# metasnv-tool/metaSNV

Hardware: AMD Instinct MI355X
Metric: pileup Gbases/s across all samples (higher is better)
Workload: dtype u8

## Files before the change

metasnv_amd/csrc/device.h:

```cpp
#pragma once

#include <cstdint>

#include <string>
#include <vector>

#include "dataset.h"

namespace msnv {

struct Pair32 { uint32_t x, y; };
struct MergedGroupDev { uint64_t hdr_base; uint32_t tile, pair_lo, n_pairs, n_pieces; };

constexpr uint8_t ANN_GENE_MINUS = 1, ANN_GENE_LINEAR = 2;
struct AnnGene   { int64_t start; int32_t contig; uint32_t flags; };
struct AnnContig { int64_t cg_base, cg_len; uint32_t goff, pad; };
struct AnnHost {
    std::vector<uint32_t> seg_beg, seg_end;
    std::vector<int32_t>  seg_gene;
    std::vector<AnnGene>  genes;
    std::vector<AnnContig> contigs;
    std::vector<uint8_t>  codons;
};
struct AnnDev {
    uint32_t *seg_beg = nullptr, *seg_end = nullptr; int32_t *seg_gene = nullptr;
    AnnGene *genes = nullptr; AnnContig *contigs = nullptr; uint8_t *codons = nullptr;
    uint32_t n_seg = 0;
    msnv_site_ann *out = nullptr; uint64_t cap_out = 0;
    uint32_t *err = nullptr;
    bool ready = false;
    std::string key;
    std::vector<std::string> gene_names;
};
int  ann_build(msnv_dataset &ds, const Annotation &an, AnnHost &h);
void ann_gene_names(const Annotation &an, const std::vector<std::string> &contigs, std::vector<std::string> &out);
int  dev_ann_upload(DeviceCols &d, const AnnHost &h);
int  dev_annotate(DeviceCols &d, uint32_t n_sites, uint32_t drop_gpos, void *stream, double *ms, uint32_t err_gpos[2]);

struct DeviceCols {
    ReadHdr  *hdr = nullptr;
    PieceHdr *hdr8 = nullptr;
    uint32_t *hdr4 = nullptr;
    PieceHdr *hdr8m = nullptr;
    uint32_t *tile_pair_merged = nullptr;
    uint32_t  n_work_merged = 0;
    MergedGroupDev *merged_groups = nullptr; uint32_t n_merged_groups = 0;
    uint32_t *blk = nullptr;
    bool      dense = true;
    uint8_t  *seq = nullptr;
    uint8_t  *qual = nullptr;
    uint64_t *s_read_base = nullptr, *s_seq_base = nullptr;
    uint32_t *ref4 = nullptr;
    uint32_t *ref_lc = nullptr;
    TilePair *pairs = nullptr;
    uint32_t *tile_pair_start = nullptr;
    WorkItem *work = nullptr;
    ChunkDesc *chunks = nullptr;
    uint32_t *tile_vbeg = nullptr, *tile_vend = nullptr;
    uint32_t  n_tiles = 0, n_pairs = 0, n_work = 0, n_work_narrow = 0, n_samples = 0;
    uint64_t  n_reads = 0, n_seq_bytes = 0, n_chunks = 0, n_hdr8m = 0, n_blk = 0;
    uint32_t *tot = nullptr;
    uint32_t *active_tiles = nullptr;
    uint32_t  n_active_tiles = 0;
    uint8_t  *part = nullptr;
// ... 144 lines not shown
```

metasnv_amd/csrc/kernels.hip:

```cpp
#include <hip/hip_runtime.h>

#include <algorithm>
#include <cstdio>
#include <cstdlib>
#include <cstring>
#include <mutex>
#include <unordered_map>
#include <vector>

#include "device.h"

namespace msnv {

#define HIP_TRY(expr)                                                                         \
    do {                                                                                      \
        hipError_t e_ = (expr);                                                               \
        if (e_ != hipSuccess) return fail(MSNV_EHIP, "%s failed: %s", #expr, hipGetErrorString(e_)); \
    } while (0)

constexpr int LANES_PER_READ = 8;
static_assert(LANES_PER_READ * 16 == SEG_MAX, "segment pieces are sized for 8 lanes of 16 bases");

struct PileupArgs {
    const ReadHdr  *hdr;
    const uint32_t *blk;
    const PieceHdr *hdr8;
    const uint32_t *hdr4;
    const PieceHdr *hdr8m;
    uint32_t        n_narrow;
    const uint8_t  *seq;
    const uint8_t  *qual;
    const uint64_t *s_read_base, *s_seq_base;
    const uint32_t *ref4;
    const TilePair *pairs;
    const WorkItem *work;
    const ChunkDesc *chunks;
    uint32_t       *tot;
    uint8_t        *part;
    uint64_t        npos;
    uint8_t        *spill;
    uint8_t        *aspill;
    Pair32         *events;   uint32_t cap_events;
    Pair32         *overflow; uint32_t cap_overflow;
    uint32_t       *counters;
    uint32_t       *ev_count;
    uint32_t        min_baseq;
    uint32_t       *ind4;
    uint32_t       *unc_bits;
    uint32_t       *slot_dirty;
    uint32_t        min_snvs;
    uint32_t        n_fused_lo;
    int             min_cov; double min_frac;
    const uint32_t *ref_lc, *tile_vbeg, *tile_vend, *tile_stage_idx;
    TileStage      *tile_stage;
    uint32_t       *stage_ovf;
};

__device__ __forceinline__ uint32_t allele_index(uint32_t code) {
    return (code == 1u) ? 0u : (code == 2u) ? 1u : (code == 4u) ? 2u : (code == 8u) ? 3u : 4u;
}
__device__ __forceinline__ uint32_t nz_bytes(uint32_t x) {
    return (((x & 0x7f7f7f7fu) + 0x7f7f7f7fu) | x) & 0x80808080u;
}
__device__ __forceinline__ uint32_t count_nz_bytes(const uint4 a, const uint4 b) {
    return (uint32_t)__popc(nz_bytes(a.x) | nz_bytes(a.y) >> 1 | nz_bytes(a.z) >> 2 | nz_bytes(a.w) >> 3 |
                            nz_bytes(b.x) >> 4 | nz_bytes(b.y) >> 5 | nz_bytes(b.z) >> 6 | nz_bytes(b.w) >> 7);
}
__device__ __forceinline__ uint32_t nz_nibbles(uint32_t x) {
    return (((x & 0x77777777u) + 0x77777777u) | x) & 0x88888888u;
}
__device__ __forceinline__ uint32_t nibflags_to_bits(uint32_t f) {
    const uint32_t e = f & 0x08080808u, o = (f >> 4) & 0x08080808u;
    return (__builtin_amdgcn_udot4(o, 0x80200802u, __builtin_amdgcn_udot4(e, 0x40100401u, 0u, false), false)) >> 3;
}
__device__ __forceinline__ uint4 any_uint4() {
    uint4 v;
    asm volatile("" : "=v"(v.x), "=v"(v.y), "=v"(v.z), "=v"(v.w));
    return v;
}
__device__ __forceinline__ uint2 lowq_fetch(const uint8_t *qlow, const uint64_t bit) {
    uint2 v;
    __builtin_memcpy(&v, qlow + (bit >> 3), 8);
    return v;
}
__device__ __forceinline__ uint32_t lowq_bits(const uint2 v, const uint32_t shift) {
    return (uint32_t)(((unsigned long long)v.y << 32 | v.x) >> shift);
}

template <int CTRL, int ROW_MASK>
__device__ __forceinline__ int dpp_add(int x) {
    return x + __builtin_amdgcn_update_dpp(0, x, CTRL, ROW_MASK, 0xf, false);
}
__device__ __forceinline__ int wave_inclusive_scan(int x) {
    x = dpp_add<0x111, 0xf>(x);
    x = dpp_add<0x112, 0xf>(x);
    x = dpp_add<0x114, 0xf>(x);
    x = dpp_add<0x118, 0xf>(x);
    x = dpp_add<0x142, 0xa>(x);
    x = dpp_add<0x143, 0xc>(x);
    return x;
}

__device__ __forceinline__ uint32_t tot_mode_of(const WorkItem &w) { return (w.part_lo >> 1) & 3u; }
__device__ __forceinline__ void tot_add(uint32_t *tot, const uint32_t mode, const uint32_t t0, const uint32_t p, const uint32_t n0, const uint32_t n1,
                                        const uint32_t n2, const uint32_t n3) {
    uint32_t *base = tot + 4ull * t0;
    if (mode == 0u) atomicAdd(base + p, n0 | n1 << 8 | n2 << 16 | n3 << 24);
    else if (mode == 1u) {
        if (n0 | n1) atomicAdd(base + 2u * p, n0 | n1 << 16);
        if (n2 | n3) atomicAdd(base + 2u * p + 1u, n2 | n3 << 16);
    } else {
        if (n0) atomicAdd(base + 4u * p, n0);
        if (n1) atomicAdd(base + 4u * p + 1u, n1);
        if (n2) atomicAdd(base + 4u * p + 2u, n2);
        if (n3) atomicAdd(base + 4u * p + 3u, n3);
    }
}
__device__ __forceinline__ void tot_add_one(uint32_t *tile_tot, const uint32_t mode, const uint32_t p, const uint32_t x, const uint32_t n) {
    const uint32_t shpack = mode == 0u ? 0x18100800u : mode == 1u ? 0x10001000u : 0u;
    const uint32_t byte_off = ((p << mode) + (x >> (2u - mode))) * 4u;
// ... 227 lines not shown
    *reinterpret_cast<uint2 *>(&L.start[2 * tid]) = make_uint2(0u, 0u);
    *reinterpret_cast<uint2 *>(&L.end[2 * tid]) = make_uint2(0u, 0u);
    L.exc[EXC_PAD + tid] = 0ull;
    if (lane == 0) L.carry[wave] = 0u;
    if (tid == 0) L.end[TILE / 4] = 0;
    const int mine = (int)(__builtin_amdgcn_udot4(st.x, 0x01010101u, __builtin_amdgcn_udot4(st.y, 0x01010101u, 0u, false), false)) -
                     (int)(__builtin_amdgcn_udot4(en.x, 0x01010101u, __builtin_amdgcn_udot4(en.y, 0x01010101u, 0u, false), false));
    d += wave_inclusive_scan(mine) - mine;
    const uint32_t v0 = ((uint32_t)d + st.x - en.x) * 0x01010101u;
    const uint32_t v1 = ((v0 >> 24) + st.y - en.y) * 0x01010101u;
    const uint32_t c0 = v0 - ex.x, c1 = v1 - ex.y;
    tc[0] += c0 & 0x00ff00ffu; tc[1] += (c0 >> 8) & 0x00ff00ffu;
    tc[2] += c1 & 0x00ff00ffu; tc[3] += (c1 >> 8) & 0x00ff00ffu;
    if (!MERGED) *reinterpret_cast<uint2 *>(a.spill + (uint64_t)k * TILE + N_PPT * tid) = make_uint2(c0, c1);
    if (MERGED && FUSED) {
        *reinterpret_cast<uint2 *>(&L.start[2 * tid]) = make_uint2(c0, c1);
        return;
    }
    if constexpr (DA && !MERGED) {
        uint32_t *row = reinterpret_cast<uint32_t *>(a.aspill) + (uint64_t)k * TILE + N_PPT * tid;
        const uint32_t ge = (0x80u - min(a.min_snvs, 127u)) * 0x01010101u;
#pragma unroll
        for (uint32_t half = 0; half < 2u; ++half) {
            const uint4 v = *reinterpret_cast<uint4 *>(&L.al[N_PPT * tid + 4u * half]);
            const uint32_t w4[4] = {v.x, v.y, v.z, v.w};
            *reinterpret_cast<uint4 *>(row + 4u * half) = v;
            if (!(v.x | v.y | v.z | v.w)) continue;
            *reinterpret_cast<uint4 *>(&L.al[N_PPT * tid + 4u * half]) = make_uint4(0u, 0u, 0u, 0u);
            dirty = true;
            uint32_t todo = 0;
#pragma unroll
            for (uint32_t j = 0; j < 4u; ++j) todo |= (split ? w4[j] != 0u : ((((w4[j] & 0x7f7f7f7fu) + ge) | w4[j]) & 0x80808080u) != 0u) ? 1u << j : 0u;
            while (todo) {
                const uint32_t j = (uint32_t)__builtin_ctz(todo);
                todo &= todo - 1u;
                const uint32_t word = j == 0u ? w4[0] : j == 1u ? w4[1] : j == 2u ? w4[2] : w4[3];
                const uint32_t gpos = t0 + N_PPT * tid + 4u * half + j;
#pragma unroll
                for (uint32_t x = 0; x < 4u; ++x) {
                    const uint32_t n = (word >> (8u * x)) & 0xffu;
                    if (n >= a.min_snvs) atomicOr(&a.ind4[gpos >> 3], 1u << (4u * (gpos & 7u) + x));
                    else if (n && split) atomicOr(&a.unc_bits[gpos >> 5], 1u << (gpos & 31u));
                }
            }
        }
        return;
    }
    uint32_t pm = 0, myev;
    {
        const uint4 a0 = *reinterpret_cast<uint4 *>(&L.al[N_PPT * tid]);
        const uint4 a1 = *reinterpret_cast<uint4 *>(&L.al[N_PPT * tid + 4]);
        const uint32_t alw[N_PPT] = {a0.x, a0.y, a0.z, a0.w, a1.x, a1.y, a1.z, a1.w};
#pragma unroll
        for (int j = 0; j < N_PPT; ++j) pm |= (alw[j] ? 1u : 0u) << j;
        myev = count_nz_bytes(a0, a1);
    }
    if (!__any(pm != 0u)) return;
    dirty |= pm != 0u;
    if (MERGED) {
        while (pm) {
            const uint32_t j = (uint32_t)__builtin_ctz(pm);
            pm &= pm - 1u;
            const uint32_t word = L.al[N_PPT * tid + j];
            L.al[N_PPT * tid + j] = 0u;
            const uint32_t gpos = t0 + N_PPT * tid + j;
            for (uint32_t m = nz_bytes(word); m; m &= m - 1u) {
                const uint32_t x = (uint32_t)__builtin_ctz(m) >> 3;
                const uint32_t n = (word >> (8u * x)) & 0xffu;
                tot_add_one(a.tot + 4ull * t0, tmode, N_PPT * tid + j, x, n);
                if (n >= a.min_snvs) atomicOr(&a.unc_bits[gpos >> 5], 1u << (gpos & 31u));
            }
        }
        return;
    }
    const uint32_t ei = (uint32_t)wave_inclusive_scan((int)myev);
    uint32_t res = 0;
    if (lane == 63 && ei) {
        uint32_t cur = atomicAdd(&L.evn, 0u);
        for (;;) {
            if (cur + ei > (uint32_t)N_EVCAP) { res = 0x80000000u | atomicAdd(a.ev_count, ei); break; }
            const uint32_t seen = atomicCAS(&L.evn, cur, cur + ei);
            if (seen == cur) { res = cur; break; }
            cur = seen;
        }
    }
    res = (uint32_t)__builtin_amdgcn_readlane((int)res, 63);
    const bool direct = (res & 0x80000000u) != 0u;
    uint32_t slot = (res & 0x7fffffffu) + ei - myev;
    while (pm) {
        const uint32_t j = (uint32_t)__builtin_ctz(pm);
        pm &= pm - 1u;
        const uint32_t word = L.al[N_PPT * tid + j];
        L.al[N_PPT * tid + j] = 0u;
        const uint32_t gpos = t0 + N_PPT * tid + j;
        for (uint32_t m = nz_bytes(word); m; m &= m - 1u) {
            const uint32_t x = (uint32_t)__builtin_ctz(m) >> 3;
            const uint32_t n = (word >> (8u * x)) & 0xffu;
            tot_add_one(a.tot + 4ull * t0, tmode, N_PPT * tid + j, x, n);
            if (n >= a.min_snvs) atomicOr(&a.ind4[gpos >> 3], 1u << (4u * (gpos & 7u) + x));
            else if (split) atomicOr(&a.unc_bits[gpos >> 5], 1u << (gpos & 31u));
            const Pair32 e{gpos, sample << 18 | x << 16 | n};
            if (direct) { if (slot < a.cap_events) a.events[slot] = e; }
            else L.ev[slot] = e;
            ++slot;
        }
    }
}

// ... 561 lines not shown
        desc_refill(L.desc, a.chunks + w.chunk_lo, c, nch, tid);
        if (L.evn >= (uint32_t)(N_EVCAP / 2)) flush_events<DenseLds, N_NT, N_EVCAP>(L, a, tid);

        const uint8_t *seq = a.seq + cd.seq_base;
        const uint64_t qbit0 = 2ull * cd.seq_base;
        uint4 sq[ROUNDS]; uint2 ql[ROUNDS];
#pragma unroll
        for (int r = 0; r < ROUNDS; ++r) {
            const uint32_t b = (uint32_t)(r * N_NT + tid);
            sq[r] = any_uint4(); ql[r] = make_uint2(0u, 0u);
            if (b < nblk) {
                ql[r] = lowq_fetch(a.qual, qbit0 + 32ull * b);
                sq[r] = *reinterpret_cast<const uint4 *>(seq + 16ull * b);
            }
        }
#pragma unroll
        for (int r = 0; r < ROUNDS; ++r) {
            if (!__any((uint32_t)(r * N_NT + tid) < nblk)) continue;
            const uint32_t d = dcur[r];
            const uint32_t P0A = d & 2047u, nA = (d >> 11) & 63u, PBv = (d >> 17) & 0xfffu;
            const bool hasB = PBv != BLK_NO_B;
            const uint32_t sB = (nA + 1u) & ~1u;
            if (d & BLK_START_A) atomicAdd(&L.start[P0A >> 2], 1u << (8u * (P0A & 3u)));
            if (d & BLK_END_A) { const uint32_t e = P0A + nA; atomicAdd(&L.end[e >> 2], 1u << (8u * (e & 3u))); }
            if (d != BLK_EMPTY && (P0A >> 9) != ((P0A + nA) >> 9)) atomicAdd(&L.carry[(P0A + nA) >> 9], 1u);
            if (hasB) {
                const uint32_t s = PBv + sB - 32u;
                if ((s >> 9) != (PBv >> 9)) atomicAdd(&L.carry[PBv >> 9], 1u);
                atomicAdd(&L.start[s >> 2], 1u << (8u * (s & 3u)));
                if (d & BLK_END_B) { const uint32_t e = PBv; atomicAdd(&L.end[e >> 2], 1u << (8u * (e & 3u))); }
            }
            const uint32_t lq = lowq_bits(ql[r], (uint32_t)qbit0 & 7u);
            dense_segment(L, sq[r], lq, P0A + 32u, 0, (int)nA);
            if (__any(hasB)) dense_segment(L, sq[r], lq, hasB ? PBv : 32u, hasB ? (int)sB : 32, 32);
        }
        if (last_chunk) {
            __syncthreads();
            narrow_pass<DenseLds, D_PAD>(L, a, tc, dirty, t0, tid, lane, wave, cd.sample, cd.pair, cd.pad, tot_mode_of(w));
        }
    }
    __syncthreads();
    flush_events<DenseLds, N_NT, N_EVCAP>(L, a, tid);
    store_part_row(a.part, w, tc, tid);
    store_item_dirty(a.slot_dirty, w, dirty, tid);
}

constexpr int GATE_NT = 256;
constexpr int GATE_PPT = TILE / GATE_NT;
static_assert(GATE_PPT == 8, "the gate kernel is written for 8 positions per thread (one site_bits word per 8 lanes)");

struct CellMap { const uint32_t *tile_site_base; const unsigned long long *tile_cell_base; const uint32_t *tile_nslots; unsigned long long cap_cells;
                 const unsigned long long *block_row; };
__device__ __forceinline__ uint64_t cell_of(const CellMap &m, const uint32_t tile, const uint32_t site, const uint32_t slot) {
    return m.tile_cell_base[tile] + (uint64_t)(site - m.tile_site_base[tile]) * m.tile_nslots[tile] + slot;
}

template <int NT>
__device__ __forceinline__ void zero_span(uint8_t *p, const uint64_t n, const uint32_t tid) {
    const uint64_t head = min(n, (uint64_t)((16u - (uint32_t)(reinterpret_cast<uintptr_t>(p) & 15u)) & 15u));
    if ((uint64_t)2u * tid < head) *reinterpret_cast<uint16_t *>(p + 2u * tid) = 0;
    uint8_t *q = p + head;
    const uint64_t body = (n - head) >> 4;
    const uint4 z = make_uint4(0u, 0u, 0u, 0u);
    for (uint64_t i = tid; i < body; i += NT) reinterpret_cast<uint4 *>(q)[i] = z;
    const uint64_t tail0 = head + (body << 4);
    if (tail0 + 2u * tid < n) *reinterpret_cast<uint16_t *>(p + tail0 + 2u * tid) = 0;
}

template <int NT>
__device__ __forceinline__ void zero_cells(uint16_t *ncol, uint16_t *cov_col, const unsigned long long cap_cells, const unsigned long long first, const unsigned long long n, const uint32_t tid) {
    if (n <= (unsigned long long)NT) {
        if (tid < (uint32_t)n) {
#pragma unroll
            for (int x = 0; x < 4; ++x) ncol[(uint64_t)x * cap_cells + first + tid] = 0;
            cov_col[first + tid] = 0;
        }
        return;
    }
#pragma unroll
    for (int x = 0; x < 4; ++x) zero_span<NT>(reinterpret_cast<uint8_t *>(ncol + (uint64_t)x * cap_cells + first), n * sizeof(uint16_t), tid);
    zero_span<NT>(reinterpret_cast<uint8_t *>(cov_col + first), n * sizeof(uint16_t), tid);
}

struct GateTile { uint32_t tile, slot_lo, slot_16, slot_w, slot_hi, vbeg, vend, n_slots; uint64_t row0; uint32_t tot_mode, staged, pair_lo, n_plane_pairs, pad0, pad1; };

struct GateArgs {
    uint32_t *tot; const uint8_t *part; const uint64_t *slot_off; const uint32_t *tile_slot_start, *tile_slot_u16, *tile_slot_wide; uint64_t npos;
    const uint32_t *tile_vbeg, *tile_vend; int min_cov, min_snvs; double min_frac;
    uint32_t *ind4, *unc_bits;
    const uint32_t *ref4, *ref_lc;
    unsigned long long *site_bits; uint32_t *site_rank; SiteRec *sites; uint32_t cap_sites; uint32_t *counters, *counters_next;
    uint32_t *tile_site_base, *tile_site_cnt; const uint32_t *active_tiles;
    uint16_t *ncol; uint16_t *cov_col; uint8_t *site_flags; uint32_t cap_out;
    const uint32_t *tile_nslots; unsigned long long *tile_cell_base; unsigned long long cap_cells;
    const GateTile *gate_tiles; uint32_t *tile_dirty; uint32_t *unc_sites; uint32_t use_dirty; unsigned long long *block_row;
    uint8_t *site_elig; uint32_t any_split;
    uint32_t n_active, tiles_per_wg;
    const TileStage *tile_stage;
    const uint8_t *aspill;
    uint32_t zero_next;
    const uint32_t *tile_list;
    uint32_t solo_cells;
};

constexpr uint32_t GATE_STAGE = 384;
constexpr uint32_t GATE_MAX_TILES = 8;
struct GateStageTile { uint32_t tile, site_rel, total, n_slots; unsigned long long cell_rel; };
// ... 560 lines not shown
                uint32_t v[4], c[4];
#pragma unroll
                for (uint32_t u = 0; u < 4u; ++u) {
                    const uint32_t k = min(kl + 4u * u, kB - 1u);
                    v[u] = rows[(uint64_t)k * TILE + off];
                    c[u] = (a.pairs[ps + k].pad >> 8) - GA_SLOTS * b;
                }
#pragma unroll
                for (uint32_t u = 0; u < 4u; ++u) {
                    if (kl + 4u * u >= kB || v[u] == 0u) continue;
#pragma unroll
                    for (uint32_t x = 0; x < 4u; ++x) {
                        const uint32_t n = (v[u] >> (8u * x)) & 0xffu;
                        if (n) atomicAdd(&s_acc[lane * GA_ROW + x * (GA_SLOTS / 2u) + (c[u] >> 1)], n << (16u * (c[u] & 1u)));
                    }
                }
            }
            __syncthreads();
            for (uint32_t idx = tid; idx < nS * 16u; idx += 256u) {
                const uint32_t row = idx >> 4, x = (idx >> 2) & 3u, seg = idx & 3u, c0 = GA_SLOTS * b + 8u * seg;
                if (c0 >= n_real) continue;
                const uint2 lo = *reinterpret_cast<const uint2 *>(&s_acc[row * GA_ROW + x * (GA_SLOTS / 2u) + 4u * seg]);
                const uint2 hi = *reinterpret_cast<const uint2 *>(&s_acc[row * GA_ROW + x * (GA_SLOTS / 2u) + 4u * seg + 2u]);
                uint16_t *dst = a.ncol + (uint64_t)x * a.cells.cap_cells + cell0 + (uint64_t)(j_lo + jj0 + row) * stride + c0;
                if (c0 + 8u <= wide_end) *reinterpret_cast<uint4 *>(dst) = make_uint4(lo.x, lo.y, hi.x, hi.y);
                else {
                    const uint32_t w[4] = {lo.x, lo.y, hi.x, hi.y};
                    for (uint32_t q = 0; q < 8u && c0 + q < n_real; ++q) dst[q] = (uint16_t)(w[q >> 1] >> (16u * (q & 1u)));
                }
            }
        }
    }
}

__device__ __forceinline__ void put_allele_word(const TailArgs &a, const uint32_t word, const unsigned long long cell, const bool add) {
    if (word == 0u) return;
#pragma unroll
    for (uint32_t x = 0; x < 4u; ++x) {
        const uint32_t n = (word >> (8u * x)) & 0xffu;
        if (!n) continue;
        uint16_t *dst = a.ncol + (uint64_t)x * a.cells.cap_cells + cell;
        if (add) add_u16(dst, n); else *dst = (uint16_t)n;
    }
}

constexpr uint32_t TAIL_POOL_WORDS = 64 * GA_ROW + 64 + 64 + 2 * GW_MAX_BLOCKS + 2;
__device__ __forceinline__ void gather_cov_block(const TailArgs &a, const uint32_t bid, uint32_t *s_pool) {
    const uint32_t GATHER_SPLIT = a.gather_split;
    const uint32_t tile = a.active_tiles[bid / GATHER_SPLIT], part = bid % GATHER_SPLIT;
    const uint32_t n = a.tile_site_cnt[tile];
    if (n <= part) return;
    const uint32_t base = a.tile_site_base[tile];
    if (base + n > a.cap_out) return;
    const uint32_t n_slots = a.cells.tile_nslots[tile];
    const unsigned long long cell0 = a.cells.tile_cell_base[tile];
    if (cell0 + (unsigned long long)n * n_slots > a.cells.cap_cells) return;
    const uint32_t ps = a.tile_pair_start[tile], np = a.tile_pair_merged[tile] - ps;
    if (np == 0u) return;
    const uint32_t t0 = tile * TILE;
    const uint32_t mine = (n - part + GATHER_SPLIT - 1) / GATHER_SPLIT;
    const uint32_t share = (n + GATHER_SPLIT - 1) / GATHER_SPLIT;
    const uint32_t *arows = a.aspill ? reinterpret_cast<const uint32_t *>(a.aspill) + (uint64_t)ps * TILE : nullptr;
    if (share >= GD_MIN_SITES) {
        const uint32_t j_lo = min(n, part * share), dense_n = min(n, j_lo + share) - j_lo;
        uint32_t *const s_lds = s_pool;
        static_assert(GA_ROW >= GW_ROW && GW_SITES == 64 && 64 * GW_ROW * 4 >= 64 * GD_ROW, "the coverage forms live in the allele gather's LDS block");
        uint32_t *const s_off = s_pool + 64 * GA_ROW, *const s_pad = s_off + 64, *const s_blk = s_pad + 64;
        if ((n_slots & 7u) == 0u && (cell0 & 7ull) == 0ull && !a.has_wide && n_slots <= 64u * GW_MAX_BLOCKS) {
            const bool has_merged = a.tile_pair_merged[tile] < a.tile_pair_start[tile + 1u];
            gather_cov_wide(a, s_lds, s_off, s_blk, t0, base, n_slots, cell0, ps, np, has_merged, j_lo, dense_n);
            if (arows) gather_alleles_wide(a, s_lds, s_off, s_blk, t0, base, n_slots, cell0, ps, np, has_merged, j_lo, dense_n);
            return;
        }
        uint8_t (*s_t)[GD_ROW] = reinterpret_cast<uint8_t (*)[GD_ROW]>(s_lds);
        const int lane = threadIdx.x & 63, wave = threadIdx.x >> 6;
        for (uint32_t jj0 = 0; jj0 < dense_n; jj0 += 64) {
            const uint32_t nS = min(64u, dense_n - jj0);
            __syncthreads();
            if (threadIdx.x < 64) s_off[threadIdx.x] = a.sites[base + j_lo + jj0 + min(threadIdx.x, nS - 1u)].gpos - t0;
            for (uint32_t kk0 = 0; kk0 < np; kk0 += 64u) {
                const uint32_t nP = min(64u, np - kk0);
                __syncthreads();
                if (threadIdx.x < nP) s_pad[threadIdx.x] = a.pairs[ps + kk0 + threadIdx.x].pad;
                const uint32_t off = s_off[lane];
                for (uint32_t kl = (uint32_t)wave; kl < nP; kl += 16) {
                    uint8_t v[4];
#pragma unroll
                    for (uint32_t u = 0; u < 4; ++u) v[u] = a.spill[(uint64_t)(ps + kk0 + min(kl + 4u * u, nP - 1u)) * TILE + off];
#pragma unroll
                    for (uint32_t u = 0; u < 4; ++u) if (kl + 4u * u < nP) s_t[lane][kl + 4u * u] = v[u];
                }
                __syncthreads();
                if ((uint32_t)lane < nP) {
                    const uint32_t pad = s_pad[lane];
                    for (uint32_t sl = (uint32_t)wave; sl < nS; sl += 4) {
                        const uint32_t cov = s_t[sl][lane];
                        uint16_t *dst = &a.cov_col[cell0 + (uint64_t)(j_lo + jj0 + sl) * n_slots + (pad >> 8)];
                        if (pad & 0xffu) add_u16(dst, cov);
                        else if (cov != 255u) *dst = (uint16_t)cov;
                    }
                }
            }
        }
        if (arows) {
            const uint64_t work = (uint64_t)dense_n * np;
            for (uint64_t i = threadIdx.x; i < work; i += blockDim.x) {
                const uint32_t j = j_lo + (uint32_t)(i / np), kk = (uint32_t)(i % np);
                const uint32_t pad = a.pairs[ps + kk].pad;
                put_allele_word(a, arows[(uint64_t)kk * TILE + (a.sites[base + j].gpos - t0)], cell0 + (uint64_t)j * n_slots + (pad >> 8), (pad & 0xffu) != 0u);
            }
        }
        return;
    }
    const uint64_t work = (uint64_t)mine * np;
    for (uint64_t i = threadIdx.x; i < work; i += blockDim.x) {
        const uint32_t j = part + (uint32_t)(i / np) * GATHER_SPLIT, kk = (uint32_t)(i % np);
        const uint32_t off = a.sites[base + j].gpos - t0;
        const uint32_t pad = a.pairs[ps + kk].pad;
        const uint32_t cov = a.spill[(uint64_t)(ps + kk) * TILE + off];
        uint16_t *dst = &a.cov_col[cell0 + (uint64_t)j * n_slots + (pad >> 8)];
        if (pad & 0xffu) add_u16(dst, cov);
        else if (cov != 255u && cov) *dst = (uint16_t)cov;
        if (arows) put_allele_word(a, arows[(uint64_t)kk * TILE + off], cell0 + (uint64_t)j * n_slots + (pad >> 8), (pad & 0xffu) != 0u);
    }
}

__device__ __forceinline__ void scatter_events_block(const TailArgs &a, const uint32_t bx, const uint32_t k) {
    if (a.counters[2] > a.cap_out || *reinterpret_cast<const unsigned long long *>(&a.counters[CNT_CELLS]) > a.cells.cap_cells) return;
    auto apply = [&](const Pair32 e, const bool allele) {
        const unsigned long long w = a.site_bits[e.x >> 6], bit = 1ull << (e.x & 63u);
        const unsigned long long row0 = a.cells.block_row[e.x >> 6];
        const uint32_t ns = a.cells.tile_nslots[e.x / TILE];
        if (!(w & bit)) return;
        const unsigned long long row = row0 + (unsigned long long)__popcll(w & (bit - 1ull)) * ns;
        if (allele) add_u16(&a.ncol[ncol_base((e.y >> 16) & 3u, a.cells.cap_cells) + row + (e.y >> 18)], e.y & 0xffffu);
        else a.cov_col[row + (e.y >> 16)] = (uint16_t)(e.y & 0xffffu);
    };
    const uint32_t n_k = min(a.counters[16u + k * EV_CNT_STRIDE], a.cap_list);
    const Pair32 *list = a.events + (uint64_t)k * a.cap_list;
    {
        constexpr uint32_t U = 4;
        const uint32_t stride = a.scatter_blocks * blockDim.x;
        uint32_t i = bx * blockDim.x + threadIdx.x;
        for (; i + (U - 1u) * stride < n_k; i += U * stride) {
            Pair32 e[U]; unsigned long long w[U], row0[U]; uint32_t ns[U];
#pragma unroll
            for (uint32_t u = 0; u < U; ++u) e[u] = list[i + u * stride];
#pragma unroll
            for (uint32_t u = 0; u < U; ++u) { w[u] = a.site_bits[e[u].x >> 6]; row0[u] = a.cells.block_row[e[u].x >> 6]; ns[u] = a.cells.tile_nslots[e[u].x / TILE]; }
#pragma unroll
            for (uint32_t u = 0; u < U; ++u) {
                const unsigned long long bit = 1ull << (e[u].x & 63u);
                if (!(w[u] & bit)) continue;
                const unsigned long long row = row0[u] + (unsigned long long)__popcll(w[u] & (bit - 1ull)) * ns[u];
                add_u16(&a.ncol[ncol_base((e[u].y >> 16) & 3u, a.cells.cap_cells) + row + (e[u].y >> 18)], e[u].y & 0xffffu);
            }
        }
        for (; i < n_k; i += stride) apply(list[i], true);
    }
    const uint32_t n_overflow = min(a.counters[1], a.cap_overflow);
    for (uint32_t i = (k * a.scatter_blocks + bx) * blockDim.x + threadIdx.x; i < n_overflow; i += a.scatter_blocks * EV_LISTS * blockDim.x)
        apply(a.overflow[i], false);
}

static bool merged_wave_form(const DeviceCols &d);
constexpr uint32_t GM_CELLS = 2048;
constexpr uint32_t GMW_CELLS = 256, GMW_PAIRS = 16, GMW_GROUPS = 4;
constexpr uint32_t GMW_HITS = 240, GM_HITS = 480;
constexpr uint32_t GMW_WORDS = 2 * (TILE / 64) + TILE / 64 + GMW_CELLS / 2 + GMW_CELLS + GMW_PAIRS + 2 + 2 * GMW_HITS;
constexpr uint32_t GM_WORDS = 2 * (TILE / 64) + TILE / 64 + GM_CELLS / 2 + GM_CELLS + MERGE_MAX_PAIRS + 2 + 2 * GM_HITS;
template <uint32_t NT, uint32_t CELLS, uint32_t PAIRS, uint32_t HITS>
__device__ __forceinline__ void gather_merged_group(const TailArgs &a, const MergedGroupDev w, uint32_t *s_tab, const uint32_t tid) {
    static_assert(GM_WORDS <= TAIL_POOL_WORDS && GMW_GROUPS * GMW_WORDS <= TAIL_POOL_WORDS && GMW_WORDS % 2 == 0, "the merged gather's tables fit the launch's LDS pool");
    static_assert((2 * (TILE / 64) + TILE / 64 + CELLS / 2 + CELLS + PAIRS + 2) % 2 == 0, "the overlap list starts on 8 bytes");
    unsigned long long *const s_bits = reinterpret_cast<unsigned long long *>(s_tab);
    uint32_t *const s_rank = s_tab + 2 * (TILE / 64);
    uint32_t *const s_cov = s_rank + TILE / 64;
    uint32_t *const s_al = s_cov + CELLS / 2;
    uint32_t *const s_gsample = s_al + CELLS;
    uint32_t *const s_nhit = s_gsample + PAIRS;
    unsigned long long *const s_hit = reinterpret_cast<unsigned long long *>(s_nhit + 2);
    auto sync = [] {
        if constexpr (NT == 64) { __builtin_amdgcn_fence(__ATOMIC_RELEASE, "wavefront"); __builtin_amdgcn_wave_barrier(); __builtin_amdgcn_fence(__ATOMIC_ACQUIRE, "wavefront"); }
        else __syncthreads();
    };
    const uint32_t tile = w.tile, t0 = tile * TILE;
    const uint32_t n = a.tile_site_cnt[tile], base = a.tile_site_base[tile], n_slots = a.cells.tile_nslots[tile];
    const unsigned long long cell0 = a.cells.tile_cell_base[tile];
    unsigned long long my_bits = 0; uint32_t my_rank = 0;
    if (tid < TILE / 64) { my_bits = a.site_bits[(t0 >> 6) + tid]; my_rank = a.site_rank[(t0 >> 6) + tid]; }
    constexpr uint32_t PF = NT == 64 ? 4u : 1u;
    PieceHdr h_first[PF];
#pragma unroll
    for (uint32_t k = 0; k < PF; ++k) { h_first[k] = PieceHdr{0u, 0u}; if (tid + k * NT < w.n_pieces) h_first[k] = a.hdr8m[w.hdr_base + tid + k * NT]; }
    const uint32_t m = w.n_pairs;
    uint32_t my_slot = 0;
    if (tid < m) my_slot = a.pairs[w.pair_lo + tid].pad >> 8;
    if (n == 0u) return;
    if (base + n > a.cap_out) return;
    if (cell0 + (unsigned long long)n * n_slots > a.cells.cap_cells) return;
    if (tid < TILE / 64) { s_bits[tid] = my_bits; s_rank[tid] = my_rank - base; }
    if (tid < m) s_gsample[tid] = my_slot;
    uint32_t my_tally = 0;
    auto count_hit = [&](const unsigned long long rec) {
        const unsigned long long qbit = rec & ((1ull << 40) - 1ull);
        const uint32_t gp = t0 + ((uint32_t)(rec >> 40) & (TILE - 1u)), cell = (uint32_t)(rec >> 51);
        const bool counted_q = !((a.qual[qbit >> 3] >> (qbit & 7u)) & 1u);
        const uint32_t code = (a.seq[qbit >> 1] >> (4u * (uint32_t)(qbit & 1u))) & 0xfu;
        const uint32_t rc = (a.ref4[gp >> 3] >> (4u * (gp & 7u))) & 0xfu;
        if (counted_q && (code == rc || (code != 0u && (code & (code - 1u)) == 0u))) {
            atomicAdd(&s_cov[cell >> 1], 1u << (16u * (cell & 1u)));
            if (code != rc) atomicAdd(&s_al[cell], 1u << (8u * (uint32_t)__builtin_ctz(code)));
        }
    };
    {
        const uint32_t n_pieces = w.n_pieces;
        const uint32_t batch = max(1u, CELLS / m);
        for (uint32_t j0 = 0; j0 < n; j0 += batch) {
            const uint32_t nj = min(batch, n - j0);
            if (tid == 0u) *s_nhit = 0u;
            for (uint32_t i = tid; i < (nj * m + 1u) / 2u; i += NT) s_cov[i] = 0u;
            for (uint32_t i = tid; i < nj * m; i += NT) s_al[i] = 0u;
            sync();
            for (uint32_t pi = tid, k = 0; pi < n_pieces; pi += NT, ++k) {
                PieceHdr h;
                if (PF == 4u) h = k == 0u ? h_first[0] : k == 1u ? h_first[PF > 1 ? 1 : 0] : k == 2u ? h_first[PF > 2 ? 2 : 0] : k == 3u ? h_first[PF > 3 ? 3 : 0] : a.hdr8m[w.hdr_base + pi];
                else h = k == 0u ? h_first[0] : a.hdr8m[w.hdr_base + pi];
                const uint32_t s = h.w0 & (TILE - 1u), len = (h.w0 >> 11) & 0xffu, pidx = (h.w0 >> 19) & 0xffu;
                const uint64_t so = ((uint64_t)(h.w0 >> 27) << 32 | h.seqoff8) << SEQ_ALIGN_LOG2;
                for (uint32_t wd = s >> 6; wd <= (s + len - 1u) >> 6 && wd < TILE / 64; ++wd) {
                    unsigned long long bits = s_bits[wd];
                    if (wd == (s >> 6)) bits &= ~0ull << (s & 63u);
                    if (wd == ((s + len - 1u) >> 6)) bits &= ~0ull >> (63u - ((s + len - 1u) & 63u));
                    while (bits) {
                        const uint32_t b = (uint32_t)__builtin_ctzll(bits);
                        const unsigned long long low = bits & (0ull - bits);
                        bits ^= low;
                        const uint32_t j = s_rank[wd] + (uint32_t)__popcll(s_bits[wd] & (low - 1ull));
                        if (j < j0 || j >= j0 + nj) continue;
                        const uint32_t q = (wd << 6) + b, o = q - s;
// ... 40 lines not shown
    if ((tid & 63u) == 0u && my_tally) atomicAdd(reinterpret_cast<unsigned long long *>(&a.counters[CNT_TALLY]), (unsigned long long)my_tally << 32);
}
__device__ __forceinline__ void gather_merged_block(const TailArgs &a, const uint32_t bid, uint32_t *s_pool) {
    if (a.merged_per_block == 1u) { gather_merged_group<256, GM_CELLS, MERGE_MAX_PAIRS, GM_HITS>(a, a.merged_groups[bid], s_pool, threadIdx.x); return; }
    const uint32_t gi = bid * GMW_GROUPS + (threadIdx.x >> 6);
    if (gi < a.n_merged_run) gather_merged_group<64, GMW_CELLS, GMW_PAIRS, GMW_HITS>(a, a.merged_groups[gi], s_pool + (threadIdx.x >> 6) * GMW_WORDS, threadIdx.x & 63u);
}
static bool merged_wave_form(const DeviceCols &d) {
    const int forced = knob::merged_gather();
    return d.max_group_pairs <= GMW_PAIRS && forced != 1;
}

template <bool HAS_MERGED>
__global__ __launch_bounds__(256) void msnv_gather_scatter(TailArgs a) {
    const uint32_t n_scatter = a.scatter_blocks * EV_LISTS;
    if (blockIdx.x == gridDim.x - 1u) {
        if (threadIdx.x < 64) {
            const uint32_t c = threadIdx.x < EV_LISTS ? a.counters[16u + threadIdx.x * EV_CNT_STRIDE] : 0u;
            unsigned long long total = c; uint32_t fullest = c;
#pragma unroll
            for (int o = 32; o >= 1; o >>= 1) { total += __shfl_xor(total, o); fullest = max(fullest, (uint32_t)__shfl_xor((int)fullest, o)); }
            if (fullest > a.cap_list) total = (unsigned long long)fullest * EV_LISTS;
            if (threadIdx.x == 0) a.counters[0] = (uint32_t)min(total, 0xffffffffull);
        }
        return;
    }
    __shared__ __attribute__((aligned(16))) uint32_t s_pool[TAIL_POOL_WORDS];
    if (blockIdx.x < n_scatter) { if (!(a.debug_skip & 1u)) scatter_events_block(a, blockIdx.x % a.scatter_blocks, blockIdx.x / a.scatter_blocks); }
    else if (HAS_MERGED && blockIdx.x < n_scatter + a.n_merged_blocks) { if (!(a.debug_skip & 4u)) gather_merged_block(a, blockIdx.x - n_scatter, s_pool); }
    else if (!(a.debug_skip & 2u)) gather_cov_block(a, blockIdx.x - n_scatter - a.n_merged_blocks, s_pool);
}

__global__ __launch_bounds__(256) void msnv_decide_sites(const SiteRec *sites, const uint32_t *unc_sites, uint32_t *counters, uint32_t cap_sites, uint32_t cap_out,
                                                         const uint32_t *ref4, const uint32_t *ref_lc, const uint16_t *ncol,
                                                         const CellMap cells, int min_snvs, double min_frac, uint8_t *site_flags) {
    __shared__ uint32_t s_pop, s_ind;
    if (threadIdx.x == 0) { s_pop = 0; s_ind = 0; }
    __syncthreads();
    const uint32_t n_unc = min(counters[CNT_UNC], cap_sites), n_sites = counters[2];
    const int lane = threadIdx.x & 63;
    if (n_sites <= cap_sites && n_sites <= cap_out && *reinterpret_cast<const unsigned long long *>(&counters[CNT_CELLS]) <= cells.cap_cells) {
        for (uint32_t u = blockIdx.x * (blockDim.x >> 6) + (threadIdx.x >> 6); u < n_unc; u += gridDim.x * (blockDim.x >> 6)) {
            const uint32_t site = unc_sites[u];
            const SiteRec s = sites[site];
            const uint32_t rc = (ref4[s.gpos >> 3] >> (4 * (s.gpos & 7))) & 0xfu;
            const bool lc = (ref_lc[s.gpos >> 5] >> (s.gpos & 31)) & 1u;
            uint32_t pop = 0, ind = 0;
            for (int x = 0; x < 4; ++x) {
                if (lc && rc == (1u << x)) continue;
                const uint32_t nx = s.n[x];
                if ((int)nx < min_snvs) continue;
                if ((double)nx >= (double)(int)s.cov * min_frac) { pop |= 1u << x; continue; }
                bool any = false;
                const uint32_t tile = s.gpos / TILE, n_slots = cells.tile_nslots[tile];
                const uint64_t row = cell_of(cells, tile, site, 0u);
                for (uint32_t i = lane; i < n_slots; i += 64)
                    any |= (int)ncol[(uint64_t)x * cells.cap_cells + row + i] >= min_snvs;
                if (__any(any)) ind |= 1u << x;
            }
            if (lane == 0) {
                site_flags[site] = (uint8_t)(pop | ind << 4);
                if (pop) atomicAdd(&s_pop, 1u);
                if (ind) atomicAdd(&s_ind, 1u);
            }
        }
    }
    __syncthreads();
    if (threadIdx.x == 0) {
        if (s_pop) atomicAdd(&counters[4], s_pop);
        if (s_ind) atomicAdd(&counters[5], s_ind);
    }
}

constexpr int C_NT = 64;
static_assert(C_NT / 64 * COV_PW == COV_ITEM_PAIRS, "coverage work items are sized for COV_PW pairs per wavefront");

__device__ __forceinline__ int wave_reduce_add(int x) {
    x = wave_inclusive_scan(x);
    return __builtin_amdgcn_readlane(x, 63);
}
__device__ __forceinline__ uint32_t row_sum16(uint32_t x) {
    x = (uint32_t)dpp_add<0xB1, 0xf>((int)x);
    x = (uint32_t)dpp_add<0x4E, 0xf>((int)x);
    x = (uint32_t)dpp_add<0x141, 0xf>((int)x);
    x = (uint32_t)dpp_add<0x140, 0xf>((int)x);
    return x;
}

template <bool WIDE>
__global__ __launch_bounds__(C_NT) void msnv_coverage_tiles(const Pair32 *iv, const TilePair *pairs,
                                                            const WorkItem *work, const uint32_t *tile_len,
                                                            unsigned long long *acc, uint32_t n_rows, int max_cov, uint32_t n_copies,
                                                            const uint64_t n_iv) {
    constexpr int WPL = WIDE ? 32 : 16;
    constexpr int LSTRIDE = WPL + 4;
    constexpr uint32_t EMPTY = WIDE ? 0u : 0x80008000u;
    __shared__ __attribute__((aligned(16))) uint32_t s_d[C_NT / 64][64 * LSTRIDE];
    __shared__ uint32_t s_mask[C_NT / 64][TILE / 32];
    const WorkItem w = work[blockIdx.x];
    const uint32_t t0 = w.tile * TILE, tl = tile_len[w.tile];
    const int lane = threadIdx.x & 63, wave = threadIdx.x >> 6;
    uint32_t *const d = s_d[wave];
    uint32_t *const mask = s_mask[wave];
    static_assert(TILE / 32 == 64, "one mask word per lane");
    auto base_of = [](const TilePair &p) -> uint64_t { return (uint64_t)p.nblk << 32 | p.blk_lo; };
    uint4 *const mine = reinterpret_cast<uint4 *>(d + LSTRIDE * lane);
    auto diff_at = [&](const uint32_t bpos) -> int {
// ... 710 lines not shown
```

metasnv_amd/csrc/pack.cpp:

```cpp
#include <algorithm>
#include <atomic>
#include <chrono>
#include <climits>
#include <cstdlib>
#include <cstring>
#include <mutex>
#include <queue>
#include <thread>
#include <unordered_map>

#include "device.h"
#include "devpack.h"
#if defined(__SSE2__)
#include <emmintrin.h>
#endif

namespace msnv {

constexpr uint32_t seq_align = SEQ_ALIGN;

static void pack_lowq(const uint8_t *q, size_t n, int cutoff, std::vector<uint8_t> &out) {
    out.assign((n + 7) / 8, 0);
    const int c_eff = std::min(std::max(cutoff, -127), 127);
    const bool all = cutoff > 127;
// ... 1020 lines not shown
            uint64_t tiles_with_pairs = 0;
            for (uint64_t t = 0; t < nt; ++t) tiles_with_pairs += tps[t + 1] > tps[t];
            const char forced = knob::fuse();
            const bool sparse = tiles_with_pairs && pairs.size() < 4 * tiles_with_pairs;
            const bool fuse_on = can_merge && forced != '0' && (sparse || forced == '1');
            const uint32_t fuse_pieces = knob::fuse_pieces();
            if (fuse_on) for (uint64_t t = 0; t < nt; ++t) {
                const uint32_t n = tps[t + 1] - tps[t];
                if (n == 0 || n > MERGE_MAX_PAIRS) continue;
                uint64_t depth = 0; bool ok = true;
                for (uint32_t k = tps[t]; k < tps[t + 1] && ok; ++k) { depth += pairs[k].max_depth; ok = !pairs[k].pad && pairs[k].read_hi - pairs[k].read_lo <= fuse_pieces; }
                if (ok && depth <= MERGE_MAX_DEPTH) fuse_tile[t] = 1;
            }
        }
        if (can_merge) {
            uint64_t shallow_pieces_total = 0, all_pieces = 0;
            for (uint64_t t = 0; t < nt; ++t) {
                uint32_t n_shallow = 0; uint64_t np = 0;
                for (uint32_t k = tps[t]; k < tps[t + 1]; ++k) { all_pieces += pairs[k].read_hi - pairs[k].read_lo; if (is_shallow(pairs[k])) { ++n_shallow; np += pairs[k].read_hi - pairs[k].read_lo; } }
                if (n_shallow >= 2) { merge_tile[t] = 1; shallow_pieces_total += np; }
            }
            const bool force = knob::merge_always();
            if (!force && shallow_pieces_total * 100 < all_pieces * 3) std::fill(merge_tile.begin(), merge_tile.end(), 0);
        }
        for (uint64_t t = 0; t < nt; ++t) {
            auto b = pairs.begin() + tps[t], e = pairs.begin() + tps[t + 1];
            if (fuse_tile[t]) for (auto it = b; it != e; ++it) it->pad = 2;
            else if (merge_tile[t]) for (auto it = b; it != e; ++it) if (is_shallow(*it)) it->pad = 2;
            auto cls = [](const TilePair &p) { return p.pad == 2 ? 2 : p.max_depth < NARROW_MAX_DEPTH ? 0 : 1; };
            bool in_class_order = true;
            for (auto it = b; it != e && it + 1 != e; ++it) if (cls(*(it + 1)) < cls(*it)) { in_class_order = false; break; }
            if (!in_class_order) std::stable_sort(b, e, [&](const TilePair &x, const TilePair &y) { return cls(x) < cls(y); });
        }
    }
    std::vector<uint32_t> tpm(nt + 1, 0);
    for (uint64_t t = 0; t < nt; ++t) { uint32_t k = tps[t]; while (k < tps[t + 1] && pairs[k].pad != 2) ++k; tpm[t] = k; }
    lap("pair CSR, merge / fuse classes");
    ds.tile_slot_base.assign(nt + 1, 0);
    ds.slot_sample.clear();
    {
        std::vector<uint32_t> nslots(nt + 1, 0);
        for (uint64_t t = 0; t < nt; ++t) {
            ds.tile_slot_base[t] = (uint64_t)ds.slot_sample.size();
            uint32_t n = 0;
            for (uint32_t k = tps[t]; k < tps[t + 1]; ++k) {
                const bool same = k > tps[t] && pairs[k].pad == 1 && (pairs[k - 1].pad & 0xffu) == 1 && pairs[k].sample == pairs[k - 1].sample;
                if (!same) { ds.slot_sample.push_back(pairs[k].sample); ++n; }
                pairs[k].pad |= (n - 1u) << 8;
            }
            nslots[t] = n >= 16u ? (n + 7u) & ~7u : n;
        }
        ds.tile_slot_stride = nslots;
        ds.tile_slot_base[nt] = (uint64_t)ds.slot_sample.size();
        if (int rc = arena.add(&d->tile_nslots, nslots, &d->device_bytes)) return rc;
        if (int rc = dev_alloc((void **)&d->tile_cell_base, (nt + 1) * sizeof(unsigned long long), &d->device_bytes)) return rc;
        if (int rc = dev_memset_async(d->tile_cell_base, 0, (nt + 1) * sizeof(unsigned long long), ds.ctx ? ds.ctx->stream : nullptr)) return rc;
    }
    lap("slots");
    std::vector<WorkItem> work;
    struct MergedGroup { uint32_t pair_lo, pair_hi, tile; };
    std::vector<MergedGroup> groups;
    {
        uint64_t total_reads_in_pairs = 0;
        for (const TilePair &p : pairs) total_reads_in_pairs += p.read_hi - p.read_lo;
        uint64_t target = knob::item_pieces();
        std::vector<WorkItem> wide, merged;
        auto chunks_of = [&](const TilePair &q) -> uint64_t {
            const bool nar = q.max_depth < NARROW_MAX_DEPTH;
            if (dense && nar) return (q.nblk + DENSE_CHUNK_BLOCKS - 1) / DENSE_CHUNK_BLOCKS;
            return (q.read_hi - q.read_lo + CHUNK_READS - 1) / CHUNK_READS;
        };
        const bool taper = knob::item_taper();
        const knob::TaperAt at = knob::taper_at();
        const double u1 = at.u1, u2 = at.u2, u3 = at.u3;
        const uint64_t base_target = target;
        const double wave_pieces = (double)dev_resident_workgroups(7) * (double)base_target;
        uint64_t seen = 0;
        for (uint64_t t = 0; t < nt; ++t) {
            uint32_t lo = tps[t];
            uint64_t acc = 0, nch = 0;
            if (taper && total_reads_in_pairs) {
                const double left = (double)(total_reads_in_pairs - seen) / wave_pieces;
                target = left < u3 ? std::max<uint64_t>(64, base_target / 8) : left < u2 ? std::max<uint64_t>(64, base_target / 4) : left < u1 ? std::max<uint64_t>(64, base_target / 2) : base_target;
            }
            {
                uint32_t g_lo = tpm[t], i_lo = tpm[t];
                uint64_t g_depth = 0, i_pieces = 0, i_chunks = 0, g_pieces = 0;
                for (uint32_t k = tpm[t]; k < tps[t + 1]; ++k) {
                    const uint32_t nr = pairs[k].read_hi - pairs[k].read_lo;
                    seen += nr;
                    if (k > g_lo && (g_depth + pairs[k].max_depth > MERGE_MAX_DEPTH || k - g_lo >= MERGE_MAX_PAIRS)) {
                        groups.push_back(MergedGroup{g_lo, k, (uint32_t)t});
                        i_pieces += g_pieces; i_chunks += (g_pieces + CHUNK_READS - 1) / CHUNK_READS;
                        g_lo = k; g_depth = 0; g_pieces = 0;
                        if (i_pieces >= target || i_chunks >= MAX_CHUNKS_PER_ITEM / 2) { merged.push_back(WorkItem{(uint32_t)t, i_lo, k, 0, 0, 0, 0, 0, ChunkDesc{}}); i_lo = k; i_pieces = 0; i_chunks = 0; }
                    }
                    g_depth += pairs[k].max_depth; g_pieces += nr;
                }
                if (tps[t + 1] > g_lo) { groups.push_back(MergedGroup{g_lo, tps[t + 1], (uint32_t)t}); merged.push_back(WorkItem{(uint32_t)t, i_lo, tps[t + 1], 0, 0, 0, 0, 0, ChunkDesc{}}); }
            }
            for (uint32_t k = tps[t]; k < tpm[t]; ++k) {
                const uint32_t nr = pairs[k].read_hi - pairs[k].read_lo;
                seen += nr;
                acc += nr; nch += chunks_of(pairs[k]);
                const bool narrow = pairs[k].max_depth < NARROW_MAX_DEPTH;
                const bool boundary = k + 1 == tpm[t] || (narrow != (pairs[k + 1].max_depth < NARROW_MAX_DEPTH));
// ... 413 lines not shown
```

Baseline: 3594.

## Flag split-slot tiles, use plain stores in scatter, restructure few-site gather

Tiles whose slots hold split pairs are now marked with a high bit in tile_nslots. The event scatter can then use a plain 16-bit store instead of an atomic add when no slot is shared, and every reader masks the flag off. The few-site gather is rebuilt so that each thread owns a pair and a stride of sites, with site offsets cached in LDS and four loads batched before the stores, replacing a div/mod indexed loop. The nonzero-byte count in the pileup now uses msad_u8, and the scatter remainder loop is folded into the unrolled loop with guarded indices. The risks are a missed mask at some nslots reader and the plain store racing when the split flag is wrong.

Result: faster. 3713 (median of 6 runs) (+3.3%).

```diff
diff --git a/metasnv_amd/csrc/device.h b/metasnv_amd/csrc/device.h
--- a/metasnv_amd/csrc/device.h
+++ b/metasnv_amd/csrc/device.h
@@ -10,6 +10,7 @@
 namespace msnv {
 
 struct Pair32 { uint32_t x, y; };
+constexpr uint32_t NSLOTS_SPLIT = 1u << 31, NSLOTS_MASK = NSLOTS_SPLIT - 1u;
 struct MergedGroupDev { uint64_t hdr_base; uint32_t tile, pair_lo, n_pairs, n_pieces; };
 
 constexpr uint8_t ANN_GENE_MINUS = 1, ANN_GENE_LINEAR = 2;
diff --git a/metasnv_amd/csrc/kernels.hip b/metasnv_amd/csrc/kernels.hip
--- a/metasnv_amd/csrc/kernels.hip
+++ b/metasnv_amd/csrc/kernels.hip
@@ -62,10 +62,6 @@
 __device__ __forceinline__ uint32_t nz_bytes(uint32_t x) {
     return (((x & 0x7f7f7f7fu) + 0x7f7f7f7fu) | x) & 0x80808080u;
 }
-__device__ __forceinline__ uint32_t count_nz_bytes(const uint4 a, const uint4 b) {
-    return (uint32_t)__popc(nz_bytes(a.x) | nz_bytes(a.y) >> 1 | nz_bytes(a.z) >> 2 | nz_bytes(a.w) >> 3 |
-                            nz_bytes(b.x) >> 4 | nz_bytes(b.y) >> 5 | nz_bytes(b.z) >> 6 | nz_bytes(b.w) >> 7);
-}
 __device__ __forceinline__ uint32_t nz_nibbles(uint32_t x) {
     return (((x & 0x77777777u) + 0x77777777u) | x) & 0x88888888u;
 }
@@ -399,8 +395,10 @@
         const uint4 a1 = *reinterpret_cast<uint4 *>(&L.al[N_PPT * tid + 4]);
         const uint32_t alw[N_PPT] = {a0.x, a0.y, a0.z, a0.w, a1.x, a1.y, a1.z, a1.w};
 #pragma unroll
-        for (int j = 0; j < N_PPT; ++j) pm |= (alw[j] ? 1u : 0u) << j;
-        myev = count_nz_bytes(a0, a1);
+        for (int j = 0; j < N_PPT; ++j) pm |= min(alw[j], 1u) << j;
+        myev = 0;
+#pragma unroll
+        for (int j = 0; j < N_PPT; ++j) myev = __builtin_amdgcn_msad_u8(alw[j] + 0x01010101u, alw[j], myev);
     }
     if (!__any(pm != 0u)) return;
     dirty |= pm != 0u;
@@ -1068,7 +1066,7 @@
 struct CellMap { const uint32_t *tile_site_base; const unsigned long long *tile_cell_base; const uint32_t *tile_nslots; unsigned long long cap_cells;
                  const unsigned long long *block_row; };
 __device__ __forceinline__ uint64_t cell_of(const CellMap &m, const uint32_t tile, const uint32_t site, const uint32_t slot) {
-    return m.tile_cell_base[tile] + (uint64_t)(site - m.tile_site_base[tile]) * m.tile_nslots[tile] + slot;
+    return m.tile_cell_base[tile] + (uint64_t)(site - m.tile_site_base[tile]) * (m.tile_nslots[tile] & NSLOTS_MASK) + slot;
 }
 
 template <int NT>
@@ -1735,7 +1733,7 @@
     if (n <= part) return;
     const uint32_t base = a.tile_site_base[tile];
     if (base + n > a.cap_out) return;
-    const uint32_t n_slots = a.cells.tile_nslots[tile];
+    const uint32_t n_slots = a.cells.tile_nslots[tile] & NSLOTS_MASK;
     const unsigned long long cell0 = a.cells.tile_cell_base[tile];
     if (cell0 + (unsigned long long)n * n_slots > a.cells.cap_cells) return;
     const uint32_t ps = a.tile_pair_start[tile], np = a.tile_pair_merged[tile] - ps;
@@ -1795,55 +1793,73 @@
         }
         return;
     }
-    const uint64_t work = (uint64_t)mine * np;
-    for (uint64_t i = threadIdx.x; i < work; i += blockDim.x) {
-        const uint32_t j = part + (uint32_t)(i / np) * GATHER_SPLIT, kk = (uint32_t)(i % np);
-        const uint32_t off = a.sites[base + j].gpos - t0;
-        const uint32_t pad = a.pairs[ps + kk].pad;
-        const uint32_t cov = a.spill[(uint64_t)(ps + kk) * TILE + off];
-        uint16_t *dst = &a.cov_col[cell0 + (uint64_t)j * n_slots + (pad >> 8)];
-        if (pad & 0xffu) add_u16(dst, cov);
-        else if (cov != 255u && cov) *dst = (uint16_t)cov;
-        if (arows) put_allele_word(a, arows[(uint64_t)kk * TILE + off], cell0 + (uint64_t)j * n_slots + (pad >> 8), (pad & 0xffu) != 0u);
+    uint32_t *const s_off = s_pool;
+    static_assert(GD_MIN_SITES <= TAIL_POOL_WORDS, "the site offsets of the few-site gather live in the launch's LDS pool");
+    const uint32_t tid = threadIdx.x;
+    const uint32_t lg = np > 1u ? min(8u, 32u - (uint32_t)__clz((int)(np - 1u))) : 0u, P = 1u << lg, S = 256u >> lg;
+    const uint32_t kk0 = tid & (P - 1u), s0 = tid >> lg;
+    const uint32_t pad0 = kk0 < np ? a.pairs[ps + kk0].pad : 0u;
+    if (tid < mine) s_off[tid] = a.sites[base + part + tid * GATHER_SPLIT].gpos - t0;
+    __syncthreads();
+    for (uint32_t kk = kk0; kk < np; kk += P) {
+        const uint32_t pad = kk == kk0 ? pad0 : a.pairs[ps + kk].pad;
+        const bool add = (pad & 0xffu) != 0u;
+        const uint8_t *row = a.spill + (uint64_t)(ps + kk) * TILE;
+        for (uint32_t jj = s0; jj < mine; jj += 4u * S) {
+            uint32_t off[4], cov[4], aw[4];
+#pragma unroll
+            for (uint32_t u = 0; u < 4u; ++u) {
+                off[u] = s_off[min(jj + u * S, mine - 1u)];
+                cov[u] = row[off[u]];
+                aw[u] = arows ? arows[(uint64_t)kk * TILE + off[u]] : 0u;
+            }
+#pragma unroll
+            for (uint32_t u = 0; u < 4u; ++u) {
+                if (jj + u * S >= mine) continue;
+                const unsigned long long cell = cell0 + (unsigned long long)(part + (jj + u * S) * GATHER_SPLIT) * n_slots + (pad >> 8);
+                if (add) { if (cov[u]) add_u16(&a.cov_col[cell], cov[u]); }
+                else if (cov[u] != 255u && cov[u]) a.cov_col[cell] = (uint16_t)cov[u];
+                if (arows) put_allele_word(a, aw[u], cell, add);
+            }
+        }
     }
 }
 
 __device__ __forceinline__ void scatter_events_block(const TailArgs &a, const uint32_t bx, const uint32_t k) {
     if (a.counters[2] > a.cap_out || *reinterpret_cast<const unsigned long long *>(&a.counters[CNT_CELLS]) > a.cells.cap_cells) return;
-    auto apply = [&](const Pair32 e, const bool allele) {
-        const unsigned long long w = a.site_bits[e.x >> 6], bit = 1ull << (e.x & 63u);
-        const unsigned long long row0 = a.cells.block_row[e.x >> 6];
-        const uint32_t ns = a.cells.tile_nslots[e.x / TILE];
-        if (!(w & bit)) return;
-        const unsigned long long row = row0 + (unsigned long long)__popcll(w & (bit - 1ull)) * ns;
-        if (allele) add_u16(&a.ncol[ncol_base((e.y >> 16) & 3u, a.cells.cap_cells) + row + (e.y >> 18)], e.y & 0xffffu);
-        else a.cov_col[row + (e.y >> 16)] = (uint16_t)(e.y & 0xffffu);
+    auto cell_at = [](const uint32_t gpos, const unsigned long long w, const unsigned long long row0, const uint32_t ns, unsigned long long &row) {
+        const unsigned long long bit = 1ull << (gpos & 63u);
+        row = row0 + (unsigned long long)__popcll(w & (bit - 1ull)) * (ns & NSLOTS_MASK);
+        return (w & bit) != 0ull;
     };
     const uint32_t n_k = min(a.counters[16u + k * EV_CNT_STRIDE], a.cap_list);
     const Pair32 *list = a.events + (uint64_t)k * a.cap_list;
     {
         constexpr uint32_t U = 4;
         const uint32_t stride = a.scatter_blocks * blockDim.x;
-        uint32_t i = bx * blockDim.x + threadIdx.x;
-        for (; i + (U - 1u) * stride < n_k; i += U * stride) {
+        for (uint32_t i = bx * blockDim.x + threadIdx.x; i < n_k; i += U * stride) {
             Pair32 e[U]; unsigned long long w[U], row0[U]; uint32_t ns[U];
 #pragma unroll
-            for (uint32_t u = 0; u < U; ++u) e[u] = list[i + u * stride];
+            for (uint32_t u = 0; u < U; ++u) e[u] = list[i + u * stride < n_k ? i + u * stride : i];
 #pragma unroll
             for (uint32_t u = 0; u < U; ++u) { w[u] = a.site_bits[e[u].x >> 6]; row0[u] = a.cells.block_row[e[u].x >> 6]; ns[u] = a.cells.tile_nslots[e[u].x / TILE]; }
 #pragma unroll
             for (uint32_t u = 0; u < U; ++u) {
-                const unsigned long long bit = 1ull << (e[u].x & 63u);
-                if (!(w[u] & bit)) continue;
-                const unsigned long long row = row0[u] + (unsigned long long)__popcll(w[u] & (bit - 1ull)) * ns[u];
-                add_u16(&a.ncol[ncol_base((e[u].y >> 16) & 3u, a.cells.cap_cells) + row + (e[u].y >> 18)], e[u].y & 0xffffu);
-            }
-        }
-        for (; i < n_k; i += stride) apply(list[i], true);
-    }
+                unsigned long long row;
+                if ((u && i + u * stride >= n_k) || !cell_at(e[u].x, w[u], row0[u], ns[u], row)) continue;
+                uint16_t *dst = &a.ncol[ncol_base((e[u].y >> 16) & 3u, a.cells.cap_cells) + row + (e[u].y >> 18)];
+                if (ns[u] & NSLOTS_SPLIT) add_u16(dst, e[u].y & 0xffffu);
+                else *dst = (uint16_t)(e[u].y & 0xffffu);
+            }
+        }
+    }
+    auto apply_cov = [&](const Pair32 e) {
+        unsigned long long row;
+        if (cell_at(e.x, a.site_bits[e.x >> 6], a.cells.block_row[e.x >> 6], a.cells.tile_nslots[e.x / TILE], row)) a.cov_col[row + (e.y >> 16)] = (uint16_t)(e.y & 0xffffu);
+    };
     const uint32_t n_overflow = min(a.counters[1], a.cap_overflow);
     for (uint32_t i = (k * a.scatter_blocks + bx) * blockDim.x + threadIdx.x; i < n_overflow; i += a.scatter_blocks * EV_LISTS * blockDim.x)
-        apply(a.overflow[i], false);
+        apply_cov(a.overflow[i]);
 }
 
 static bool merged_wave_form(const DeviceCols &d);
@@ -1868,7 +1884,7 @@
         else __syncthreads();
     };
     const uint32_t tile = w.tile, t0 = tile * TILE;
-    const uint32_t n = a.tile_site_cnt[tile], base = a.tile_site_base[tile], n_slots = a.cells.tile_nslots[tile];
+    const uint32_t n = a.tile_site_cnt[tile], base = a.tile_site_base[tile], n_slots = a.cells.tile_nslots[tile] & NSLOTS_MASK;
     const unsigned long long cell0 = a.cells.tile_cell_base[tile];
     unsigned long long my_bits = 0; uint32_t my_rank = 0;
     if (tid < TILE / 64) { my_bits = a.site_bits[(t0 >> 6) + tid]; my_rank = a.site_rank[(t0 >> 6) + tid]; }
@@ -2015,7 +2031,7 @@
                 if ((int)nx < min_snvs) continue;
                 if ((double)nx >= (double)(int)s.cov * min_frac) { pop |= 1u << x; continue; }
                 bool any = false;
-                const uint32_t tile = s.gpos / TILE, n_slots = cells.tile_nslots[tile];
+                const uint32_t tile = s.gpos / TILE, n_slots = cells.tile_nslots[tile] & NSLOTS_MASK;
                 const uint64_t row = cell_of(cells, tile, site, 0u);
                 for (uint32_t i = lane; i < n_slots; i += 64)
                     any |= (int)ncol[(uint64_t)x * cells.cap_cells + row + i] >= min_snvs;
diff --git a/metasnv_amd/csrc/pack.cpp b/metasnv_amd/csrc/pack.cpp
--- a/metasnv_amd/csrc/pack.cpp
+++ b/metasnv_amd/csrc/pack.cpp
@@ -1096,6 +1096,8 @@
         }
         ds.tile_slot_stride = nslots;
         ds.tile_slot_base[nt] = (uint64_t)ds.slot_sample.size();
+        for (uint64_t t = 0; t < nt; ++t)
+            for (uint32_t k = tps[t]; k < tps[t + 1]; ++k) if ((pairs[k].pad & 0xffu) == 1u) { nslots[t] |= NSLOTS_SPLIT; break; }
         if (int rc = arena.add(&d->tile_nslots, nslots, &d->device_bytes)) return rc;
         if (int rc = dev_alloc((void **)&d->tile_cell_base, (nt + 1) * sizeof(unsigned long long), &d->device_bytes)) return rc;
         if (int rc = dev_memset_async(d->tile_cell_base, 0, (nt + 1) * sizeof(unsigned long long), ds.ctx ? ds.ctx->stream : nullptr)) return rc;
```
